# AER-RC/RRTMG_LW

Hardware: AMD Instinct MI355X
Metric: columns/sec, 72-layer profiles (higher is better)
Workload: dtype f64 (transmittance / tfn codes and their LDS table f32); 1 GPU; 1000000 synthetic 72-layer columns, config 'cloudy' (icld=2: rtrnmr max-random overlap, idrv=0), sharded 1x1000000; ncol_total=1000000, nlay=72, columns_per_gpu=1000000, parallelism=columns/1, gather=none, kdata=stand-in (real k-data absent from the reference mount), sweeps=production

## Files before the change

include/rrtmg_lw_hip.h:

```cpp
#ifndef RRTMG_LW_HIP_H
#define RRTMG_LW_HIP_H

#ifdef __cplusplus
extern "C" {
#endif

#define RRTMG_LW_HIP_OK 0
#define RRTMG_LW_HIP_EPHYSICS 1
#define RRTMG_LW_HIP_EARG 2
#define RRTMG_LW_HIP_ENODEVICE 3
#define RRTMG_LW_HIP_ENOTINIT 4
#define RRTMG_LW_HIP_EDATA 5
#define RRTMG_LW_HIP_EHIP 6

#define RRTMG_LW_NBND 16
#define RRTMG_LW_NGPT 140

int rrtmg_lw_hip_init(const char *static_tables_path, const char *kdata_path, double cpdair, int device);

int rrtmg_lw_hip_init_devices(const char *static_tables_path, const char *kdata_path, double cpdair, int ndev, const int *devices);
int rrtmg_lw_hip_num_devices(void);

int rrtmg_lw_hip_kdata_is_standin(void);

// ... 173 lines not shown
    const double *cldfr, const double *taucld, const double *cicewp, const double *cliqwp,
    const double *reice, const double *reliq, const double *tauaer,
    double *uflx, double *dflx, double *hr, double *uflxc, double *dflxc, double *hrc,
    double *duflx_dt, double *duflxc_dt);
int rrtmg_lw_hip_queue_flush(void);
int rrtmg_lw_hip_queue_columns(void);

unsigned rrtmg_lw_hip_build_flags(void);
int rrtmg_lw_hip_set_batch(int ncol_batch);
int rrtmg_lw_hip_effective_batch(int nlay);
int rrtmg_lw_hip_set_overlap(int on);
int rrtmg_lw_hip_set_cu_partition(int layer_cus);
int rrtmg_lw_hip_cu_partition(void);
int rrtmg_lw_hip_set_one_sweep_max(int ncol);
int rrtmg_lw_hip_set_split_max(int ncol);
int rrtmg_lw_hip_set_graph_max(int ncol);
void rrtmg_lw_hip_graph_stats(long long *captures, long long *replays);
int rrtmg_lw_hip_set_wide_window(int on);

int rrtmg_lw_hip_set_layer_split(int on);
int rrtmg_lw_hip_set_column_sort(int on, int min_gain);
int rrtmg_lw_hip_column_sort_min(void);
long long rrtmg_lw_hip_workspace_bytes(void);
int rrtmg_lw_hip_set_n1_prototype(int on);
int rrtmg_lw_hip_n1_prototype(void);
int rrtmg_lw_hip_num_chunks(void);
int rrtmg_lw_hip_gpoints(void);

void rrtmg_lw_hip_profile_begin(void);
int rrtmg_lw_hip_profile_end(char *buf, int len);
// ... 33 lines not shown
```

rrtmg_lw_amd/api.py:

```python
from __future__ import annotations

import ctypes as C
import os

import numpy as np

_HERE = os.path.dirname(os.path.abspath(__file__))
LIB_PATH = os.environ.get("RRTMG_LW_HIP_LIB", os.path.join(_HERE, "librrtmg_lw_hip.so"))
STATIC_BLOB = os.path.join(_HERE, "data", "lw_static.bin")
STANDIN_KDATA = os.path.join(_HERE, "data", "standin.kdata.bin")
REAL_KDATA = os.path.join(os.path.dirname(_HERE), "data", "rrtmg_lw.kdata.bin")
NBND, NGPT = 16, 140

LIB_PATH_G256 = os.path.join(_HERE, "librrtmg_lw_hip_g256.so")

_dp = C.POINTER(C.c_double)
_lib = None
_libs = {}
_gpoints = 140
_initialised = False


class RrtmgLwError(RuntimeError):
    pass
# ... 121 lines not shown
def workspace_bytes():
    lib().rrtmg_lw_hip_workspace_bytes.restype = C.c_longlong
    return int(lib().rrtmg_lw_hip_workspace_bytes())


def set_one_sweep_max(ncol):
    return int(lib().rrtmg_lw_hip_set_one_sweep_max(C.c_int(int(ncol))))


def set_layer_split(on):
    return int(lib().rrtmg_lw_hip_set_layer_split(C.c_int(1 if on else 0)))


def set_split_max(ncol):
    return int(lib().rrtmg_lw_hip_set_split_max(C.c_int(int(ncol))))


def set_graph_max(ncol):
    return int(lib().rrtmg_lw_hip_set_graph_max(C.c_int(int(ncol))))


def graph_stats():
    a, b = C.c_longlong(0), C.c_longlong(0)
    lib().rrtmg_lw_hip_graph_stats(C.byref(a), C.byref(b))
    return int(a.value), int(b.value)


def set_wide_window(on):
    return int(lib().rrtmg_lw_hip_set_wide_window(C.c_int(1 if on else 0)))

# ... 429 lines not shown
```

rrtmg_lw_amd/csrc/driver.hip:

```cpp
#include <hip/hip_runtime.h>
#include <cstdlib>
#include <sched.h>

#include <algorithm>
#include <atomic>
#include <cstdint>
#include <cstdarg>
#include <mutex>
#include <string>
#include <chrono>
#include <condition_variable>
#include <functional>
#include <map>
#include <thread>
#include <vector>

#include "../../include/rrtmg_lw_hip.h"
#include "kernels.hip"
#include "mtjump.hpp"

namespace {

using namespace rrlw;

// ... 214 lines not shown
        } else {                                                                                 \
            hipLaunchKernelGGL(KERNEL, GRID, BLOCKDIM, LDS, STREAM, __VA_ARGS__);                \
        }                                                                                        \
    } while (0)

template <int Q, bool SPEC = false>
int sweepc_attr_one()
{
#ifndef RRLW_TUNE
    HIP_TRY(hipFuncSetAttribute((const void *)k_sweepc<Q, 0, false, sweepc_nt(Q, 0, false), SPEC>, hipFuncAttributeMaxDynamicSharedMemorySize, SWEEPC_LDS_MAX));
    HIP_TRY(hipFuncSetAttribute((const void *)k_sweepc<Q, 0, true, sweepc_nt(Q, 0, true), SPEC>, hipFuncAttributeMaxDynamicSharedMemorySize, SWEEPC_LDS_MAX));
    HIP_TRY(hipFuncSetAttribute((const void *)k_sweepc<Q, 2, true, sweepc_nt(Q, 2, true), SPEC>, hipFuncAttributeMaxDynamicSharedMemorySize, SWEEPC_LDS_MAX));
#endif
    HIP_TRY(hipFuncSetAttribute((const void *)k_sweepc<Q, 1, false, sweepc_nt(Q, 1, false), SPEC>, hipFuncAttributeMaxDynamicSharedMemorySize, SWEEPC_LDS_MAX));
    HIP_TRY(hipFuncSetAttribute((const void *)k_sweepc<Q, 2, false, sweepc_nt(Q, 2, false), SPEC>, hipFuncAttributeMaxDynamicSharedMemorySize, SWEEPC_LDS_MAX));
    return 0;
}
template <int Q>
int sweepz_attr_spec()
{
#ifndef RRLW_TUNE
    HIP_TRY(hipFuncSetAttribute((const void *)k_sweepz<Q, 1, false, true>, hipFuncAttributeMaxDynamicSharedMemorySize, SWEEPC_LDS_MAX));
    HIP_TRY(hipFuncSetAttribute((const void *)k_sweepz<Q, 1, true, true>, hipFuncAttributeMaxDynamicSharedMemorySize, SWEEPC_LDS_MAX));
    HIP_TRY(hipFuncSetAttribute((const void *)k_sweepz<Q, 2, true, true>, hipFuncAttributeMaxDynamicSharedMemorySize, SWEEPC_LDS_MAX));
    HIP_TRY(hipFuncSetAttribute((const void *)k_sweepz<Q, 3, false, true>, hipFuncAttributeMaxDynamicSharedMemorySize, SWEEPC_LDS_MAX));
    HIP_TRY(hipFuncSetAttribute((const void *)k_sweepz<Q, 3, true, true>, hipFuncAttributeMaxDynamicSharedMemorySize, SWEEPC_LDS_MAX));
    HIP_TRY(hipFuncSetAttribute((const void *)k_sweepz<Q, 4, false, true>, hipFuncAttributeMaxDynamicSharedMemorySize, SWEEPC_LDS_MAX));
    HIP_TRY(hipFuncSetAttribute((const void *)k_sweepz<Q, 4, true, true>, hipFuncAttributeMaxDynamicSharedMemorySize, SWEEPC_LDS_MAX));
#endif
    HIP_TRY(hipFuncSetAttribute((const void *)k_sweepz<Q, 2, false, true>, hipFuncAttributeMaxDynamicSharedMemorySize, SWEEPC_LDS_MAX));
// ... 72 lines not shown
        const int zcap = sweepz_group_cap(nq, idrv == 1);
        const int cap = std::max(1, std::min(sweepc_group_cap(nq), mode != 0 ? zcap : 99));
        for (int k0 = 0; k0 < nbs[nq]; k0 += cap) {
            if (fg.n >= NGROUP_MAX) return false;
            const int nbg = std::min(cap, nbs[nq] - k0);
            fg.nb[fg.n] = nbg;
            fg.bands[fg.n] = (lists[nq] >> (4 * k0)) & (nbg >= 16 ? ~0ull : ((1ull << (4 * nbg)) - 1ull));
            fg.gq[fg.n++] = nq;
        }
    }
    return true;
}

void graphs_clear();
int g_split_max = []() { const char *e = getenv("RRTMG_LW_SPLIT_MAX"); return e ? std::max(0, atoi(e)) : 768; }();
int ensure_workspace(int nlay, int ncolb, bool cloud, bool mc = false, int idrv = 1, int mode = -1)
{
    SweepGroups fgw;
    int groups = NGROUP_MAX;
    if (mode >= 0 && make_groups(mode, idrv, 1, NBND, fgw)) groups = fgw.n;
    const bool gdp = idrv == 1, efcl = cloud && (mode < 0 || mode == 1 || mode == 3), ovl = cloud && (mode < 0 || mode == 2);
    const size_t split_cols = ncolb <= g_split_max ? (size_t)NBND * align_up((size_t)ncolb, 64) : 0;
    if (G.ws_base && G.ws_nlay == nlay && G.ws_ncolb >= ncolb && (G.ws_cloud || !cloud) && (G.ws_mc || !mc) && (G.ws_two_scr || !G.split_sweep) &&
        G.ws_groups >= groups && G.ws_slabcols >= split_cols && (G.ws_gdp || !gdp) && (G.ws_efcl || !efcl) && (G.ws_ovl || !ovl)) return 0;
    if (G.ws_base) { HIP_TRY(hipDeviceSynchronize()); graphs_clear(); HIP_TRY(hipFree(G.ws_base)); G.ws_base = nullptr; }
    const bool same = G.ws_nlay == nlay;
    ncolb = std::max(ncolb, same ? G.ws_ncolb : 0);
    cloud = cloud || G.ws_cloud || mc;
    mc = mc || G.ws_mc;
    const int ng = std::max(groups, G.ws_groups);
// ... 285 lines not shown
    sa.tlay = GCM ? g.tlay : c.tavel;
    sa.tlev = GCM ? g.tlev : c.tz;
    const bool spec = GCM && out.uflxs;
    sa.uflxs = spec ? out.uflxs : nullptr; sa.dflxs = spec ? out.dflxs : nullptr;
    sa.uflxcs = spec ? out.uflxcs : nullptr; sa.dflxcs = spec ? out.dflxcs : nullptr;
    SweepGroups fg;
    if (!make_groups(mode, idrv, istart, iend, fg)) return fail(RRTMG_LW_HIP_EARG, "internal: more than %d sweep groups", NGROUP_MAX);
    if ((!split && fg.n > G.ws_groups) || (idrv == 1 && !G.ws_gdp)) return fail(RRTMG_LW_HIP_EARG, "internal: workspace holds %d band groups, the call needs %d", G.ws_groups, fg.n);
    const int *gq = fg.gq;
    int slab0[NGROUP_MAX];
    unsigned long long gsz = 0ull;
    { int sl = 0; for (int g = 0; g < fg.n; g++) { slab0[g] = sl; const int n = split ? fg.nb[g] : 1; gsz |= (unsigned long long)n << (4 * g); sl += n; } }
#define SWEEPC_I(Q, PH, I)                                                                                           \
    do {                                                                                                             \
        constexpr int nt = sweepc_nt(Q, PH, I);                                                                      \
        const int wnb = split ? 1 : sa.nbands;                                             \
        const int nsb = split ? 1 : sweepc_nsb(Q, PH, I, sa.nbands);                                                 \
        sa.ncb = (nb + 64 * nsb - 1) / (64 * nsb);                                                                   \
        const dim3 sgrid((unsigned)sa.ncb, split ? sa.nbands : 1), sblock(64, wnb * nt, nsb);                        \
        if (spec) LAUNCH_LDS("k_sweepc<" #Q "," #PH ",spec>", (k_sweepc<Q, PH, I, nt, true>), sgrid, sblock, sweepc_lds_bytes(PH, I, wnb, nsb, nt), s, G.D, Wk, sa); \
        else LAUNCH_LDS("k_sweepc<" #Q "," #PH ">", (k_sweepc<Q, PH, I, nt>), sgrid, sblock, sweepc_lds_bytes(PH, I, wnb, nsb, nt), s, G.D, Wk, sa); \
    } while (0)
#ifdef RRLW_TUNE
#define SWEEPC(Q, PH) do { if (idrv == 1) return fail(RRTMG_LW_HIP_EARG, "tuning build: idrv = 0 only"); else SWEEPC_I(Q, PH, false); } while (0)
#else
#define SWEEPC(Q, PH) do { if (idrv == 1 && PH != 1) SWEEPC_I(Q, PH, true); else SWEEPC_I(Q, PH, false); } while (0)
#endif
#define SWEEPC_Q(PH) do { if (nq == 4) SWEEPC(4, PH); else if (nq == 3) SWEEPC(3, PH); else if (nq == 2) SWEEPC(2, PH); else SWEEPC(1, PH); } while (0)
    for (int phase = 0; phase < 3; phase++) {
        if (phase == 1) {
            if (mode == 0) continue;
            for (int g = 0; g < fg.n; g++) {
                const int nq = gq[g];
                sa.bands = fg.bands[g];
// ... 169 lines not shown
        if (int rc = make_stream(&G.lay_m, 0, G.cu_layer)) return rc;
    }
    if (G.ev_last_valid) HIP_TRY(hipStreamWaitEvent(s, G.ev_last, 0));
    State::GraphEnt *gent = nullptr;
    bool capture = false;
    if (single && !split && !gen.on && !mc && !G.profile && !G.n1 && ncol <= g_graph_max) {
        std::vector<unsigned char> key;
        key_put(key, ncol); key_put(key, nlay); key_put(key, mode); key_put(key, idrv); key_put(key, inflag); key_put(key, iceflag); key_put(key, liqflag);
        const double *gp[] = {g.play, g.plev, g.tlay, g.tlev, g.tsfc, g.h2ovmr, g.o3vmr, g.co2vmr, g.ch4vmr, g.n2ovmr, g.o2vmr, g.cfc11vmr, g.cfc12vmr,
                              g.cfc22vmr, g.ccl4vmr, g.emis, g.cldfr, g.taucld, g.cicewp, g.cliqwp, g.reice, g.reliq, g.tauaer, g.tauctot,
                              out.uflx, out.dflx, out.hr, out.uflxc, out.dflxc, out.hrc, out.duflx_dt, out.duflxc_dt, out.fnet, out.fnetc,
                              out.uflxs, out.dflxs, out.uflxcs, out.dflxcs};
        key_put(key, gp);
        key_put(key, G.init_gen); key_put(key, G.device);
        key_put(key, G.ws_base); key_put(key, G.ws_bytes); key_put(key, g_colsort); key_put(key, g_colsort_min); key_put(key, g_one_sweep_max);
        key_put(key, g_wide_window); key_put(key, g_layer_split); key_put(key, g_prep_fork); key_put(key, G.sweep_fanout); key_put(key, eff_batch(nlay)); key_put(key, g_split_max);
        for (auto &e : G.graphs) if (e.key == key) { gent = &e; break; }
        if (!gent) {
            if (G.graphs.size() >= GRAPH_CACHE) {
                size_t old = 0;
                for (size_t j = 1; j < G.graphs.size(); j++) if (G.graphs[j].used < G.graphs[old].used) old = j;
                if (G.graphs[old].exec) (void)hipGraphExecDestroy(G.graphs[old].exec);
                G.graphs.erase(G.graphs.begin() + (long)old);
            }
            G.graphs.emplace_back();
            gent = &G.graphs.back();
            gent->key = key;
        }
        gent->used = ++G.graph_clock;
        if (gent->exec) {
            HIP_TRY(hipGraphLaunch(gent->exec, s));
// ... 1119 lines not shown
    g_graph_max = ncol < 0 ? 0 : ncol;
    return prev;
}
void rrtmg_lw_hip_graph_stats(long long *captures, long long *replays)
{
    ENTRY_LOCK;
    if (captures) *captures = g_states[0].graph_captures;
    if (replays) *replays = g_states[0].graph_replays;
}

int rrtmg_lw_hip_set_split_max(int ncol)
{
    ENTRY_LOCK;
    const int prev = g_split_max;
    g_split_max = ncol < 0 ? 0 : ncol;
    return prev;
}

int rrtmg_lw_hip_set_wide_window(int on)
{
    ENTRY_LOCK;
    const int prev = g_wide_window ? 1 : 0;
    g_wide_window = on != 0;
    return prev;
}

int rrtmg_lw_hip_set_layer_split(int on)
{
    ENTRY_LOCK;
    const int prev = g_layer_split ? 1 : 0;
// ... 1304 lines not shown
```

rrtmg_lw_amd/csrc/kernels.hip:

```cpp
#include <hip/hip_runtime.h>
#include "kissjump.hpp"

#if (defined(RRLW_KO_LDS_UNIFORM) || defined(RRLW_KO_HALFG) || defined(RRLW_KO_STORES) || defined(RRLW_KO_HALFSTORE)) && !defined(RRLW_TUNE)
#error "RRLW_KO_* knock-outs give wrong results: tuning builds (-DRRLW_TUNE) only"
#endif
#ifdef RRLW_TUNE
#define RRLW_BF_TUNE 1u
#else
#define RRLW_BF_TUNE 0u
#endif
#if defined(RRLW_KO_LDS_UNIFORM) || defined(RRLW_KO_HALFG) || defined(RRLW_KO_STORES) || defined(RRLW_KO_HALFSTORE)
#define RRLW_BF_KNOCKOUT 2u
#else
#define RRLW_BF_KNOCKOUT 0u
#endif
#if (defined(RRLW_CODE_BITS) && RRLW_CODE_BITS != 32) || defined(RRLW_DECODE_F64) || defined(RRLW_SWEEP_EXPF) || defined(RRLW_EXACT_DIV) || defined(RRLW_FDIV_TWO_NEWTON)
#define RRLW_BF_NUMERICS 4u
#else
#define RRLW_BF_NUMERICS 0u
#endif
#ifdef RRLW_G256
#define RRLW_BF_G256 8u
#else
#define RRLW_BF_G256 0u
// ... 2590 lines not shown
    const float t = (float)idx * 1.0e-4f;
    const float tau = bpade * t * __builtin_amdgcn_rcpf(1.0f - t);
    const float ex = __builtin_amdgcn_exp2f(-1.44269504088896f * tau);
    const float atr = 1.0f - ex;
    float tfn = tau < 0.06f ? tau * (1.0f / 6.0f) : 1.0f - 2.0f * (__builtin_amdgcn_rcpf(tau) - ex * __builtin_amdgcn_rcpf(atr));
    if (idx == 0u) tfn = 0.0f;
    if (idx >= 10000u) tfn = 1.0f;
    return make_float2(idx == 0u ? 0.0f : atr, tfn);
}
#ifdef RRLW_SWEEP_EXPF
#define RRLW_LUT_ENTRY(lut, idx) lut_entry_expf((idx), 3.5971223f)
#else
#define RRLW_LUT_ENTRY(lut, idx) (lut)[(idx)]
#endif

__device__ __forceinline__ double planck_at(const double *tp, const double *tq, double t)
{
    const double x = t - 159.;
    const int ind = clampi((int)x, 1, 180);
    const double f = x - (double)ind;
    return fma(f, tq[ind] - tq[ind - 1], tp[ind - 1]);
}

__device__ __forceinline__ void sweep_stage_lut(const DevTables &T, unsigned char *smem, int tid, int nth)
{
    const double2 *src = reinterpret_cast<const double2 *>(T.stat + T.sl.lutf);
    double2 *dst = reinterpret_cast<double2 *>(smem);
#ifdef RRLW_SWEEP_EXPF
    constexpr int NLUT = 0;
#else
    constexpr int NLUT = SWEEP_LUT_BYTES / 16;
#endif
    for (int i0 = tid; i0 < NLUT; i0 += 8 * nth) {
        double2 v[8];
#pragma unroll
        for (int k = 0; k < 8; k++) v[k] = src[min(i0 + k * nth, NLUT - 1)];
// ... 64 lines not shown
    return (RRLW_SWEEPC_SPLIT && NQ == 4 && (PHASE == 2 || PHASE == 0)) ? 2 : 1;
}
__host__ __device__ constexpr int sweepc_group_cap(int NQ)
{
    int cap = 5;
    for (int ph = 0; ph < 3; ph++)
        for (int i = 0; i < 2; i++) {
            if (ph == 1 && i == 1) continue;
            const bool idrv = i == 1;
            const int nt = sweepc_nt(NQ, ph, idrv), w = 4 * sweepc_waves(NQ / nt, ph, idrv) / nt;
            if (w < cap) cap = w;
            while (cap > 1 && sweepc_lds_bytes(ph, idrv, cap, 1, nt) > SWEEPC_LDS_MAX) cap--;
        }
    return cap;
}
__host__ __device__ constexpr int sweepc_nsb(int NQ, int PHASE, bool IDRV, int nb)
{
    const int nt = sweepc_nt(NQ, PHASE, IDRV);
    int nsb = nsb_fit(4 * sweepc_waves(NQ / nt, PHASE, IDRV) / (nb * nt));
    while (nsb > 1 && sweepc_lds_bytes(PHASE, IDRV, nb, nsb, nt) > SWEEPC_LDS_MAX) nsb = nsb_fit(nsb - 1);
    return nsb;
}

template <int G> struct SweepcLev { double tl, tz; unsigned w; };

__device__ __forceinline__ double one_minus(double x)
{
    double t = 1.0 - x;
    asm("" : "+v"(t));
    return t;
}
__device__ __forceinline__ double times(double x, double y)
{
    double t = x * y;
    asm("" : "+v"(t));
    return t;
}

template <int NQ, int PHASE, bool IDRV, int NT = 1, bool SPEC = false>
__global__ __launch_bounds__(256 * sweepc_waves(NQ / NT, PHASE, IDRV), sweepc_waves(NQ / NT, PHASE, IDRV)) void k_sweepc(DevTables T, Workspace W, SweepArgs a)
{
    static_assert(NQ % NT == 0 && (NT == 1 || NT == 2 || NT == 3), "threads per band");
    constexpr int G = NQ / NT, NG = 4 * G, NC = RRLW_SWEEPC_CODES;
    constexpr bool DOWN = PHASE != 2, UP = PHASE != 1, TWO = PHASE == 2;
    constexpr int NVAL = sweepc_nval(PHASE, IDRV);
    extern __shared__ __align__(16) unsigned char smem[];
    const int tx = threadIdx.x, ty = __builtin_amdgcn_readfirstlane(threadIdx.y), sub = __builtin_amdgcn_readfirstlane(threadIdx.z);
    const int bi = ty / NT, part = ty % NT;
    const int ny = blockDim.y, nb = ny / NT, nsb = blockDim.z, ncw = 64 * nsb;
    const float2 *s_lut = reinterpret_cast<const float2 *>(smem);
    double (*s_pl)[184] = reinterpret_cast<double (*)[184]>(smem + SWEEP_LUT_BYTES + bi * SWEEPC_BAND_BYTES);
    double (*s_fr)[16] = reinterpret_cast<double (*)[16]>(smem + SWEEP_LUT_BYTES + bi * SWEEPC_BAND_BYTES + SWEEP_PL_BYTES);
    double *red = reinterpret_cast<double *>(smem + SWEEP_LUT_BYTES + nb * SWEEPC_BAND_BYTES);
    const int slot = blockIdx.x * nsb + sub;
    const int cblock = PHASE == 0 ? slot : __builtin_amdgcn_readfirstlane(W.order[slot]);
    const int col = cblock * 64 + tx;
    const int bsel = a.split ? (int)blockIdx.y : 0;
    const unsigned long long bands = a.bands >> (4 * bsel);
    const int B = (int)((bands >> (4 * bi)) & 15ull) + 1;
    const bool incol = col < a.ncol;
    const int colc = incol ? col : a.ncol - 1;
    const int quad = __builtin_amdgcn_readfirstlane(band_qstart(B) + part * G);
    const int g0 = NG * part;
    const int pc = pcol(W, colc);
    const size_t gc = (size_t)a.col0 + pc;
    const int nlay = W.nlay, nct = a.nct;
    const size_t ncb = W.ncolb;
    const bool alt16 = (B == 16 && a.istart == 16);
    const bool lo_bin = (LO_BINARY >> (B - 1)) & 1u, up_bin = (UP_BINARY >> (B - 1)) & 1u;
    const bool any_bin = lo_bin || up_bin;
    const int base_up = ((UP_ZERO >> (B - 1)) & 1u) ? 14 : (((UP_FROM_A >> (B - 1)) & 1u) ? 0 : 9);
    sweep_stage_lut(T, smem, (sub * ny + ty) * 64 + tx, 64 * ny * nsb);
    sweep_stage_band(T, s_pl, s_fr, B, alt16, lo_bin, up_bin, (sub * NT + part) * 64 + tx, NT * ncw);
    __syncthreads();
    const int lo = PHASE == 0 ? 1 : __builtin_amdgcn_readfirstlane(W.hgrp[(blockIdx.x * nsb) / SORT_GROUP]) + 1;
    const size_t qstride = (size_t)nlay * ncb;
    const unsigned *__restrict__ sC = W.scr[S_CODE] + (size_t)quad * qstride * CODE_WORDS;
    const unsigned *__restrict__ sFw = W.fw + (size_t)fw_slot(B) * nlay * ncb;
    const bool moved = pmoved(W, colc);
    const double *__restrict__ tlay = moved ? W.tlayc : a.tlay + a.col0;
    const double *__restrict__ tlev = moved ? W.tlevc : a.tlev + a.col0;
    const size_t tstride = moved ? ncb : (size_t)nct;
    const unsigned offc = (unsigned)colc * (unsigned)CODE_BYTES, off8p = (unsigned)colc * 8u, off4 = (unsigned)colc * 4u;
    const size_t pcb = (size_t)W.pcb;
    const size_t gslab = (size_t)(a.group + bsel) * (nlay + 1) * pcb;
    double *__restrict__ gdn1 = W.gdn1 + gslab;
    double *__restrict__ gup1 = W.gup1 + gslab;
    Part2 *__restrict__ gup = W.gup + gslab;
    Part2 *__restrict__ gdp = W.gdp + gslab;
    const unsigned so8 = (unsigned)col * 8u, so16 = (unsigned)col * 16u;
    const int laytrop = W.laytrop[colc];
    const double *tp0 = s_pl[0], *tp1 = s_pl[1];
    double2 *hand = reinterpret_cast<double2 *>(W.hand) + ((size_t)quad * ncb + colc) * 2;
    const size_t hstream = (size_t)NQUAD * ncb * 2;

    constexpr bool SOFF = PHASE != 1;
    const unsigned ncb32 = (unsigned)ncb, tstr32 = (unsigned)tstride;
    auto fill_t = [&](auto bin_tag, int lev, int zoff, SweepcLev<G> &q) {
        const int l = min(max(lev, 1), nlay);
        if constexpr (SOFF) {
            const unsigned r = (unsigned)(l - 1);
            q.tl = bload_f64(row_ptr(tlay, r, tstr32), off8p);
            q.tz = bload_f64(row_ptr(tlev, r + (unsigned)zoff, tstr32), off8p);
            if constexpr (decltype(bin_tag)::value) q.w = bload_u32(sFw, off4, r * ncb32 * 4u);
        } else {
            q.tl = bload_f64(tlay + tstride * (l - 1), off8p);
            q.tz = bload_f64(tlev + tstride * (l - 1 + zoff), off8p);
            if constexpr (decltype(bin_tag)::value) q.w = bload_u32(sFw + (size_t)(l - 1) * ncb, off4);
        }
    };
    auto ld_c = [&](int lev, int k) -> pk4 {
        const int l = min(max(lev, 1), nlay);
        if constexpr (SOFF) return bload_pk4_nt(sC + (size_t)k * qstride * CODE_WORDS, offc, (unsigned)(l - 1) * ncb32 * (unsigned)CODE_BYTES);
        else return bload_pk4_nt(sC + ((size_t)k * qstride + (size_t)(l - 1) * ncb) * CODE_WORDS, offc);
    };
    auto frac_row = [&](int lev, unsigned fwv, double &fpl) -> const double * {
        const bool lower = lev <= laytrop;
        if (any_bin) {
            const unsigned w = (lower ? lo_bin : up_bin) ? fwv : 0x10000000u;
            const int r0 = clampi((lower ? 0 : base_up) + (int)(w >> 28) - 1, 0, 14);
            fpl = (double)(w & 0x0fffffffu) * (1.0 / 268435456.0);
            return &s_fr[r0][g0];
        }
        fpl = 0.0;
        return &s_fr[lower ? 0 : base_up][g0];
    };

    const unsigned rlane = (unsigned)(sub * 64 + tx);
    const unsigned vstride = (unsigned)(ny * NC * ncw), rband = (unsigned)(ty * NC * ncw);
    unsigned bufoff = 0u;
    auto red_put = [&](int c, int val, double v) { red[bufoff + val * vstride + rband + (unsigned)(c * ncw) + rlane] = v; };
    auto round_end = [&](auto dn_tag, int lev0, int nvalid) {
#pragma clang fp contract(off)
        constexpr bool DN = decltype(dn_tag)::value;
        constexpr int NV = DN ? 1 : NVAL;
        __syncthreads();
        for (int c = ty; c < nvalid; c += ny) {
            const int lvl = DN ? lev0 - c - 1 : lev0 + c;
            double sv[NV];
#pragma unroll
            for (int val = 0; val < NV; val++) {
                const double *r = red + (bufoff + val * vstride + (unsigned)(c * ncw) + rlane);
                const bool deriv = IDRV && !DN && val >= (TWO ? 2 : 1);
                double sum = 0.0;
                for (int q = 0; q < nb; q++) {
                    double pq = r[(unsigned)(q * NT * NC * ncw)];
// ... 19 lines not shown
                if constexpr (DN) bstore_f64(gdn1 + (size_t)lvl * pcb, so8, sv[0]);
                else {
                    if constexpr (TWO) bstore_f64x2(gup + (size_t)lvl * pcb, so16, sv[0], sv[1]);
                    else bstore_f64(gup1 + (size_t)lvl * pcb, so8, sv[0]);
                    if constexpr (IDRV) bstore_f64x2(gdp + (size_t)lvl * pcb, so16, TWO ? sv[2] : sv[1], TWO ? sv[3] : sv[1]);
                }
            }
        }
        bufoff = bufoff ? 0u : NVAL * vstride;
    };

    double rad[NG], radc[TWO ? NG : 1], drad[IDRV ? NG : 1], dradc[(IDRV && TWO) ? NG : 1];
#pragma unroll
    for (int j = 0; j < NG; j++) rad[j] = 0.0;

    SweepcLev<G> cur;
    cur.w = 0u;
    pk4 cc[G][NC];
    int ki = 0;
    auto level = [&](auto bin_tag, auto dn_tag, int lev, int slot) {
        constexpr bool BIN = decltype(bin_tag)::value, DN = decltype(dn_tag)::value;
        constexpr int dir = DN ? -1 : 1;
        ki_salu(ki);
        double fpl;
        const double *row = frac_row(lev, cur.w, fpl);
        const double blay = planck_at(tp0, tp0, cur.tl);
        const double dpl = planck_at(tp0, (DN && alt16 && lev == 1) ? tp1 : tp0, cur.tz) - blay;
        fill_t(bin_tag, lev + dir, DN ? 0 : 1, cur);
        double qs[G], qsc[G], qd[G], qdc[G];
#pragma unroll
        for (int k = 0; k < G; k++) {
            float2 e[4];
            pk4 pk;
#pragma unroll
            for (int c = 0; c < NC; c++) if (c == slot) pk = cc[k][c];
            const scr4 ck = unpack4(pk);
#pragma unroll
            for (int jj = 0; jj < 4; jj++) e[jj] = RRLW_LUT_ENTRY(s_lut, code_index(ck.v[jj]));
            {
                const pk4 nx = ld_c(lev + NC * dir, k);
#pragma unroll
                for (int c = 0; c < NC; c++) if (c == slot) cc[k][c] = nx;
            }
#pragma unroll
            for (int jj = 0; jj < 4; jj++) {
                const int j = 4 * k + jj;
                double atr, tfn;
                decode(ck.v[jj], e[jj], atr, tfn);
                double fr = row[j];
                if constexpr (BIN) fr = fma(fpl, row[16 + j] - fr, fr);
                const double bb = fr * fma(tfn, dpl, blay);
                rad[j] = fma(bb - rad[j], atr, rad[j]);
                if constexpr (TWO && !DN) radc[j] = fma(bb - radc[j], atr, radc[j]);
                if constexpr (IDRV && !DN) {
                    const double tr = one_minus(atr);
                    drad[j] = times(drad[j], tr);
                    if constexpr (TWO) dradc[j] = times(dradc[j], tr);
                }
            }
            qs[k] = (rad[4 * k] + rad[4 * k + 1]) + (rad[4 * k + 2] + rad[4 * k + 3]);
            if constexpr (TWO && !DN) qsc[k] = (radc[4 * k] + radc[4 * k + 1]) + (radc[4 * k + 2] + radc[4 * k + 3]);
            if constexpr (IDRV && !DN) {
                qd[k] = (drad[4 * k] + drad[4 * k + 1]) + (drad[4 * k + 2] + drad[4 * k + 3]);
                if constexpr (TWO) qdc[k] = (dradc[4 * k] + dradc[4 * k + 1]) + (dradc[4 * k + 2] + dradc[4 * k + 3]);
            }
            if (RRLW_SWEEPC_QUAD_BARRIER) __builtin_amdgcn_sched_barrier(0);
        }
        auto tree = [&](const double (&q)[G]) -> double {
            if constexpr (G == 1) return q[0];
            else if constexpr (G == 2) return q[0] + q[1];
            else if constexpr (G == 3) return (q[0] + q[1]) + q[2];
            else return (q[0] + q[1]) + (q[2] + q[3]);
        };
        red_put(slot, 0, tree(qs));
        if constexpr (TWO && !DN) red_put(slot, 1, tree(qsc));
        if constexpr (IDRV && !DN) {
            red_put(slot, TWO ? 2 : 1, tree(qd));
            if constexpr (TWO) red_put(slot, 3, tree(qdc));
        }
    };
    auto sweep = [&](auto bin_tag, auto dn_tag) {
        constexpr bool DN = decltype(dn_tag)::value;
        constexpr int dir = DN ? -1 : 1;
        const int first = DN ? nlay : lo, count = nlay - lo + 1;
#pragma unroll
        for (int c = 0; c < NC; c++) {
            if (c == NC - 1) fill_t(bin_tag, first, DN ? 0 : 1, cur);
#pragma unroll
            for (int k = 0; k < G; k++) cc[k][c] = ld_c(first + c * dir, k);
        }
        int n = 0;
        for (; n + NC <= count; n += NC) {
#pragma unroll
// ... 2 lines not shown
        }
        const int rem = count - n;
#pragma unroll
        for (int c = 0; c < NC - 1; c++) {
            if (c < rem) level(bin_tag, dn_tag, first + (n + c) * dir, c);
        }
        if (rem > 0) round_end(dn_tag, first + n * dir, rem);
    };
    using std::true_type;
    using std::false_type;

    if constexpr (DOWN) {
        if (incol && ty == 0) bstore_f64(gdn1 + (size_t)nlay * pcb, so8, 0.0);
        if constexpr (SPEC) {
            if (incol && part == 0) {
                const size_t o = spec_at(gc, nlay, B, nlay, nct);
                a.dflxs[o] = 0.0;
                if (a.dflxcs) a.dflxcs[o] = 0.0;
            }
        }
        if (any_bin) sweep(true_type{}, true_type{}); else sweep(false_type{}, true_type{});
    }
    if constexpr (PHASE == 1) {
        if (incol) {
#pragma unroll
            for (int k = 0; k < G; k++) {
                hand[(size_t)k * ncb * 2] = make_double2(rad[4 * k], rad[4 * k + 1]);
                hand[(size_t)k * ncb * 2 + 1] = make_double2(rad[4 * k + 2], rad[4 * k + 3]);
            }
        }
        return;
    }

    if constexpr (PHASE == 0) {
        const double reflect = 1. - a.emis[gc + (size_t)nct * (B - 1)];
        const double pb = W.percol[(size_t)(PC_PLANKBND + B - 1) * ncb + colc];
        const double dpb = IDRV ? W.percol[(size_t)(PC_DPLANKBND + B - 1) * ncb + colc] : 0.0;
        double fpl;
        const double *row = frac_row(1, any_bin ? bload_u32(sFw, off4) : 0u, fpl);
        double usum = 0.0, dusum = 0.0;
#pragma unroll
        for (int j = 0; j < NG; j++) {
            const double fr = any_bin ? fma(fpl, row[16 + j] - row[j], row[j]) : row[j];
            rad[j] = fma(reflect, rad[j], fr * pb);
            usum = usum + rad[j];
            if constexpr (IDRV) { drad[j] = times(fr, dpb); dusum = dusum + drad[j]; }
        }
        red_put(0, 0, usum);
        if constexpr (IDRV) red_put(0, 1, dusum);
        round_end(false_type{}, 0, 1);
    } else {
#pragma unroll
        for (int k = 0; k < G; k++) {
            const double2 *h = hand + (size_t)k * ncb * 2;
            const double2 a0 = h[hstream], a1 = h[hstream + 1], c0 = h[2 * hstream], c1 = h[2 * hstream + 1];
            rad[4 * k] = a0.x; rad[4 * k + 1] = a0.y; rad[4 * k + 2] = a1.x; rad[4 * k + 3] = a1.y;
            if constexpr (TWO) { radc[4 * k] = c0.x; radc[4 * k + 1] = c0.y; radc[4 * k + 2] = c1.x; radc[4 * k + 3] = c1.y; }
            if constexpr (IDRV) {
                const double2 d0 = h[3 * hstream], d1 = h[3 * hstream + 1], e0 = h[4 * hstream], e1 = h[4 * hstream + 1];
                drad[4 * k] = d0.x; drad[4 * k + 1] = d0.y; drad[4 * k + 2] = d1.x; drad[4 * k + 3] = d1.y;
                if constexpr (TWO) { dradc[4 * k] = e0.x; dradc[4 * k + 1] = e0.y; dradc[4 * k + 2] = e1.x; dradc[4 * k + 3] = e1.y; }
            }
        }
    }
    if constexpr (UP) {
        if (any_bin) sweep(true_type{}, false_type{}); else sweep(false_type{}, false_type{});
    }
}

// ... 740 lines not shown
```

Baseline: 17.27 million columns/s.

## Merge several single-quad bands per thread in the clear-sky sweep kernel

```diff
diff --git a/include/rrtmg_lw_hip.h b/include/rrtmg_lw_hip.h
--- a/include/rrtmg_lw_hip.h
+++ b/include/rrtmg_lw_hip.h
@@ -211,6 +211,7 @@
 int rrtmg_lw_hip_cu_partition(void);
 int rrtmg_lw_hip_set_one_sweep_max(int ncol);
 int rrtmg_lw_hip_set_split_max(int ncol);
+int rrtmg_lw_hip_set_band_merge(int on);
 int rrtmg_lw_hip_set_graph_max(int ncol);
 void rrtmg_lw_hip_graph_stats(long long *captures, long long *replays);
 int rrtmg_lw_hip_set_wide_window(int on);
diff --git a/rrtmg_lw_amd/api.py b/rrtmg_lw_amd/api.py
--- a/rrtmg_lw_amd/api.py
+++ b/rrtmg_lw_amd/api.py
@@ -159,6 +159,10 @@
 
 def set_split_max(ncol):
     return int(lib().rrtmg_lw_hip_set_split_max(C.c_int(int(ncol))))
+
+
+def set_band_merge(on):
+    return int(lib().rrtmg_lw_hip_set_band_merge(C.c_int(1 if on else 0)))
 
 
 def set_graph_max(ncol):
diff --git a/rrtmg_lw_amd/csrc/driver.hip b/rrtmg_lw_amd/csrc/driver.hip
--- a/rrtmg_lw_amd/csrc/driver.hip
+++ b/rrtmg_lw_amd/csrc/driver.hip
@@ -252,6 +252,15 @@
 #endif
     HIP_TRY(hipFuncSetAttribute((const void *)k_sweepc<Q, 1, false, sweepc_nt(Q, 1, false), SPEC>, hipFuncAttributeMaxDynamicSharedMemorySize, SWEEPC_LDS_MAX));
     HIP_TRY(hipFuncSetAttribute((const void *)k_sweepc<Q, 2, false, sweepc_nt(Q, 2, false), SPEC>, hipFuncAttributeMaxDynamicSharedMemorySize, SWEEPC_LDS_MAX));
+    if constexpr (!SPEC && sweepc_nbt(Q, 1, false) > 1) {
+#ifndef RRLW_TUNE
+        HIP_TRY(hipFuncSetAttribute((const void *)k_sweepc<Q, 0, false, 1, false, sweepc_nbt(Q, 0, false)>, hipFuncAttributeMaxDynamicSharedMemorySize, SWEEPC_LDS_MAX));
+        HIP_TRY(hipFuncSetAttribute((const void *)k_sweepc<Q, 0, true, 1, false, sweepc_nbt(Q, 0, true)>, hipFuncAttributeMaxDynamicSharedMemorySize, SWEEPC_LDS_MAX));
+        HIP_TRY(hipFuncSetAttribute((const void *)k_sweepc<Q, 2, true, 1, false, sweepc_nbt(Q, 2, true)>, hipFuncAttributeMaxDynamicSharedMemorySize, SWEEPC_LDS_MAX));
+#endif
+        HIP_TRY(hipFuncSetAttribute((const void *)k_sweepc<Q, 1, false, 1, false, sweepc_nbt(Q, 1, false)>, hipFuncAttributeMaxDynamicSharedMemorySize, SWEEPC_LDS_MAX));
+        HIP_TRY(hipFuncSetAttribute((const void *)k_sweepc<Q, 2, false, 1, false, sweepc_nbt(Q, 2, false)>, hipFuncAttributeMaxDynamicSharedMemorySize, SWEEPC_LDS_MAX));
+    }
     return 0;
 }
 template <int Q>
@@ -354,6 +363,8 @@
 
 void graphs_clear();
 int g_split_max = []() { const char *e = getenv("RRTMG_LW_SPLIT_MAX"); return e ? std::max(0, atoi(e)) : 768; }();
+constexpr int bands_with_quads(int nq) { int n = 0; for (int B = 1; B <= NBND; B++) n += band_nquad(B) == nq ? 1 : 0; return n; }
+bool g_band_merge = []() { const char *e = getenv("RRTMG_LW_BAND_MERGE"); return !e || atoi(e) != 0; }();
 int ensure_workspace(int nlay, int ncolb, bool cloud, bool mc = false, int idrv = 1, int mode = -1)
 {
     SweepGroups fgw;
@@ -669,10 +680,15 @@
 #define SWEEPC_I(Q, PH, I)                                                                                           \
     do {                                                                                                             \
         constexpr int nt = sweepc_nt(Q, PH, I);                                                                      \
+        constexpr int nbt = sweepc_nbt(Q, PH, I);                                 \
+        const bool merge = nbt > 1 && g_band_merge && !split && !spec && sa.nbands == bands_with_quads(Q);             \
         const int wnb = split ? 1 : sa.nbands;                                             \
-        const int nsb = split ? 1 : sweepc_nsb(Q, PH, I, sa.nbands);                                                 \
+        const int nsb = split ? 1 : sweepc_nsb(Q, PH, I, sa.nbands, merge ? nbt : 1);                                \
         sa.ncb = (nb + 64 * nsb - 1) / (64 * nsb);                                                                   \
-        const dim3 sgrid((unsigned)sa.ncb, split ? sa.nbands : 1), sblock(64, wnb * nt, nsb);                        \
+        const dim3 sgrid((unsigned)sa.ncb, split ? sa.nbands : 1), sblock(64, merge ? wnb / nbt : wnb * nt, nsb);    \
+        if constexpr (nbt > 1) {                                                                                     \
+            if (merge) { LAUNCH_LDS("k_sweepc<" #Q "," #PH ",merged>", (k_sweepc<Q, PH, I, 1, false, nbt>), sgrid, sblock, sweepc_lds_bytes(PH, I, wnb, nsb, 1), s, G.D, Wk, sa); break; } \
+        }                                                                                                            \
         if (spec) LAUNCH_LDS("k_sweepc<" #Q "," #PH ",spec>", (k_sweepc<Q, PH, I, nt, true>), sgrid, sblock, sweepc_lds_bytes(PH, I, wnb, nsb, nt), s, G.D, Wk, sa); \
         else LAUNCH_LDS("k_sweepc<" #Q "," #PH ">", (k_sweepc<Q, PH, I, nt>), sgrid, sblock, sweepc_lds_bytes(PH, I, wnb, nsb, nt), s, G.D, Wk, sa); \
     } while (0)
@@ -872,7 +888,7 @@
         key_put(key, gp);
         key_put(key, G.init_gen); key_put(key, G.device);
         key_put(key, G.ws_base); key_put(key, G.ws_bytes); key_put(key, g_colsort); key_put(key, g_colsort_min); key_put(key, g_one_sweep_max);
-        key_put(key, g_wide_window); key_put(key, g_layer_split); key_put(key, g_prep_fork); key_put(key, G.sweep_fanout); key_put(key, eff_batch(nlay)); key_put(key, g_split_max);
+        key_put(key, g_wide_window); key_put(key, g_layer_split); key_put(key, g_prep_fork); key_put(key, G.sweep_fanout); key_put(key, eff_batch(nlay)); key_put(key, g_split_max); key_put(key, g_band_merge);
         for (auto &e : G.graphs) if (e.key == key) { gent = &e; break; }
         if (!gent) {
             if (G.graphs.size() >= GRAPH_CACHE) {
@@ -2022,6 +2038,14 @@
     ENTRY_LOCK;
     const int prev = g_split_max;
     g_split_max = ncol < 0 ? 0 : ncol;
+    return prev;
+}
+
+int rrtmg_lw_hip_set_band_merge(int on)
+{
+    ENTRY_LOCK;
+    const int prev = g_band_merge ? 1 : 0;
+    g_band_merge = on != 0;
     return prev;
 }
 
diff --git a/rrtmg_lw_amd/csrc/kernels.hip b/rrtmg_lw_amd/csrc/kernels.hip
--- a/rrtmg_lw_amd/csrc/kernels.hip
+++ b/rrtmg_lw_amd/csrc/kernels.hip
@@ -2628,12 +2628,22 @@
 #define RRLW_LUT_ENTRY(lut, idx) (lut)[(idx)]
 #endif
 
+__device__ __forceinline__ void planck_idx(double t, int &ind, double &f)
+{
+    const double x = t - 159.;
+    ind = clampi((int)x, 1, 180);
+    f = x - (double)ind;
+}
+__device__ __forceinline__ double planck_eval(const double *tp, const double *tq, int ind, double f)
+{
+    return fma(f, tq[ind] - tq[ind - 1], tp[ind - 1]);
+}
 __device__ __forceinline__ double planck_at(const double *tp, const double *tq, double t)
 {
-    const double x = t - 159.;
-    const int ind = clampi((int)x, 1, 180);
-    const double f = x - (double)ind;
-    return fma(f, tq[ind] - tq[ind - 1], tp[ind - 1]);
+    int ind;
+    double f;
+    planck_idx(t, ind, f);
+    return planck_eval(tp, tq, ind, f);
 }
 
 __device__ __forceinline__ void sweep_stage_lut(const DevTables &T, unsigned char *smem, int tid, int nth)
@@ -2728,15 +2738,22 @@
         }
     return cap;
 }
-__host__ __device__ constexpr int sweepc_nsb(int NQ, int PHASE, bool IDRV, int nb)
+__host__ __device__ constexpr int sweepc_nbt(int NQ, int PHASE, bool IDRV) { (void)IDRV; return NQ != 1 ? 1 : PHASE == 1 ? 4 : 2; }
+__host__ __device__ constexpr int sweepc_waves_m(int PHASE, bool IDRV) { return PHASE == 0 && !IDRV ? 3 : 2; }
+__host__ __device__ constexpr int sweepc_waves_of(int NQ, int PHASE, bool IDRV, int NT, int NBT)
+{
+    return NBT == 1 ? sweepc_waves(NQ / NT, PHASE, IDRV) : sweepc_waves_m(PHASE, IDRV);
+}
+__host__ __device__ constexpr int sweepc_nsb(int NQ, int PHASE, bool IDRV, int nb, int NBT = 1)
 {
     const int nt = sweepc_nt(NQ, PHASE, IDRV);
-    int nsb = nsb_fit(4 * sweepc_waves(NQ / nt, PHASE, IDRV) / (nb * nt));
-    while (nsb > 1 && sweepc_lds_bytes(PHASE, IDRV, nb, nsb, nt) > SWEEPC_LDS_MAX) nsb = nsb_fit(nsb - 1);
+    int nsb = NBT == 1 ? nsb_fit(4 * sweepc_waves(NQ / nt, PHASE, IDRV) / (nb * nt))
+                       : nsb_fit(4 * sweepc_waves_m(PHASE, IDRV) / (nb / NBT));
+    while (nsb > 1 && sweepc_lds_bytes(PHASE, IDRV, nb, nsb, NBT == 1 ? nt : 1) > SWEEPC_LDS_MAX) nsb = nsb_fit(nsb - 1);
     return nsb;
 }
 
-template <int G> struct SweepcLev { double tl, tz; unsigned w; };
+template <int NB> struct SweepcLev { double tl, tz; unsigned w[NB]; };
 
 __device__ __forceinline__ double one_minus(double x)
 {
@@ -2751,46 +2768,59 @@
     return t;
 }
 
-template <int NQ, int PHASE, bool IDRV, int NT = 1, bool SPEC = false>
-__global__ __launch_bounds__(256 * sweepc_waves(NQ / NT, PHASE, IDRV), sweepc_waves(NQ / NT, PHASE, IDRV)) void k_sweepc(DevTables T, Workspace W, SweepArgs a)
+template <int NQ, int PHASE, bool IDRV, int NT = 1, bool SPEC = false, int NBT = 1>
+__global__ __launch_bounds__(256 * sweepc_waves_of(NQ, PHASE, IDRV, NT, NBT), sweepc_waves_of(NQ, PHASE, IDRV, NT, NBT)) void k_sweepc(DevTables T, Workspace W, SweepArgs a)
 {
     static_assert(NQ % NT == 0 && (NT == 1 || NT == 2 || NT == 3), "threads per band");
-    constexpr int G = NQ / NT, NG = 4 * G, NC = RRLW_SWEEPC_CODES;
+    static_assert(NBT == 1 || (NT == 1 && !SPEC), "several bands per thread: whole bands, no spectral outputs");
+    constexpr int G = NQ * NBT / NT, NG = 4 * G, QB = G / NBT, NC = RRLW_SWEEPC_CODES;
     constexpr bool DOWN = PHASE != 2, UP = PHASE != 1, TWO = PHASE == 2;
     constexpr int NVAL = sweepc_nval(PHASE, IDRV);
     extern __shared__ __align__(16) unsigned char smem[];
     const int tx = threadIdx.x, ty = __builtin_amdgcn_readfirstlane(threadIdx.y), sub = __builtin_amdgcn_readfirstlane(threadIdx.z);
-    const int bi = ty / NT, part = ty % NT;
-    const int ny = blockDim.y, nb = ny / NT, nsb = blockDim.z, ncw = 64 * nsb;
+    const int bi = (ty / NT) * NBT, part = ty % NT;
+    const int ny = blockDim.y, nb = (ny / NT) * NBT, nsb = blockDim.z, ncw = 64 * nsb;
     const float2 *s_lut = reinterpret_cast<const float2 *>(smem);
-    double (*s_pl)[184] = reinterpret_cast<double (*)[184]>(smem + SWEEP_LUT_BYTES + bi * SWEEPC_BAND_BYTES);
-    double (*s_fr)[16] = reinterpret_cast<double (*)[16]>(smem + SWEEP_LUT_BYTES + bi * SWEEPC_BAND_BYTES + SWEEP_PL_BYTES);
     double *red = reinterpret_cast<double *>(smem + SWEEP_LUT_BYTES + nb * SWEEPC_BAND_BYTES);
     const int slot = blockIdx.x * nsb + sub;
     const int cblock = PHASE == 0 ? slot : __builtin_amdgcn_readfirstlane(W.order[slot]);
     const int col = cblock * 64 + tx;
     const int bsel = a.split ? (int)blockIdx.y : 0;
     const unsigned long long bands = a.bands >> (4 * bsel);
-    const int B = (int)((bands >> (4 * bi)) & 15ull) + 1;
     const bool incol = col < a.ncol;
     const int colc = incol ? col : a.ncol - 1;
-    const int quad = __builtin_amdgcn_readfirstlane(band_qstart(B) + part * G);
     const int g0 = NG * part;
     const int pc = pcol(W, colc);
     const size_t gc = (size_t)a.col0 + pc;
     const int nlay = W.nlay, nct = a.nct;
     const size_t ncb = W.ncolb;
-    const bool alt16 = (B == 16 && a.istart == 16);
-    const bool lo_bin = (LO_BINARY >> (B - 1)) & 1u, up_bin = (UP_BINARY >> (B - 1)) & 1u;
-    const bool any_bin = lo_bin || up_bin;
-    const int base_up = ((UP_ZERO >> (B - 1)) & 1u) ? 14 : (((UP_FROM_A >> (B - 1)) & 1u) ? 0 : 9);
+    int B[NBT], quad[NBT], base_up[NBT];
+    bool alt16[NBT], lo_bin[NBT], up_bin[NBT], any_bin = false;
+    double (*s_pl[NBT])[184];
+    double (*s_fr[NBT])[16];
     sweep_stage_lut(T, smem, (sub * ny + ty) * 64 + tx, 64 * ny * nsb);
-    sweep_stage_band(T, s_pl, s_fr, B, alt16, lo_bin, up_bin, (sub * NT + part) * 64 + tx, NT * ncw);
+#pragma unroll
+    for (int kb = 0; kb < NBT; kb++) {
+        B[kb] = (int)((bands >> (4 * (bi + kb))) & 15ull) + 1;
+        quad[kb] = __builtin_amdgcn_readfirstlane(band_qstart(B[kb]) + part * G);
+        alt16[kb] = (B[kb] == 16 && a.istart == 16);
+        lo_bin[kb] = (LO_BINARY >> (B[kb] - 1)) & 1u;
+        up_bin[kb] = (UP_BINARY >> (B[kb] - 1)) & 1u;
+        any_bin = any_bin || lo_bin[kb] || up_bin[kb];
+        base_up[kb] = ((UP_ZERO >> (B[kb] - 1)) & 1u) ? 14 : (((UP_FROM_A >> (B[kb] - 1)) & 1u) ? 0 : 9);
+        s_pl[kb] = reinterpret_cast<double (*)[184]>(smem + SWEEP_LUT_BYTES + (bi + kb) * SWEEPC_BAND_BYTES);
+        s_fr[kb] = reinterpret_cast<double (*)[16]>(smem + SWEEP_LUT_BYTES + (bi + kb) * SWEEPC_BAND_BYTES + SWEEP_PL_BYTES);
+        sweep_stage_band(T, s_pl[kb], s_fr[kb], B[kb], alt16[kb], lo_bin[kb], up_bin[kb], (sub * NT + part) * 64 + tx, NT * ncw);
+    }
     __syncthreads();
     const int lo = PHASE == 0 ? 1 : __builtin_amdgcn_readfirstlane(W.hgrp[(blockIdx.x * nsb) / SORT_GROUP]) + 1;
     const size_t qstride = (size_t)nlay * ncb;
-    const unsigned *__restrict__ sC = W.scr[S_CODE] + (size_t)quad * qstride * CODE_WORDS;
-    const unsigned *__restrict__ sFw = W.fw + (size_t)fw_slot(B) * nlay * ncb;
+    const unsigned *sC[NBT], *sFw[NBT];
+#pragma unroll
+    for (int kb = 0; kb < NBT; kb++) {
+        sC[kb] = W.scr[S_CODE] + (size_t)quad[kb] * qstride * CODE_WORDS;
+        sFw[kb] = W.fw + (size_t)(NBT == 1 ? fw_slot(B[kb]) : min(fw_slot(B[kb]), NFW - 1)) * nlay * ncb;
+    }
     const bool moved = pmoved(W, colc);
     const double *__restrict__ tlay = moved ? W.tlayc : a.tlay + a.col0;
     const double *__restrict__ tlev = moved ? W.tlevc : a.tlev + a.col0;
@@ -2804,46 +2834,52 @@
     Part2 *__restrict__ gdp = W.gdp + gslab;
     const unsigned so8 = (unsigned)col * 8u, so16 = (unsigned)col * 16u;
     const int laytrop = W.laytrop[colc];
-    const double *tp0 = s_pl[0], *tp1 = s_pl[1];
-    double2 *hand = reinterpret_cast<double2 *>(W.hand) + ((size_t)quad * ncb + colc) * 2;
+    auto hand_at = [&](int k) -> double2 * { return reinterpret_cast<double2 *>(W.hand) + ((size_t)(quad[k / QB] + k % QB) * ncb + colc) * 2; };
     const size_t hstream = (size_t)NQUAD * ncb * 2;
 
     constexpr bool SOFF = PHASE != 1;
     const unsigned ncb32 = (unsigned)ncb, tstr32 = (unsigned)tstride;
-    auto fill_t = [&](auto bin_tag, int lev, int zoff, SweepcLev<G> &q) {
+    auto fill_t = [&](auto bin_tag, int lev, int zoff, SweepcLev<NBT> &q) {
         const int l = min(max(lev, 1), nlay);
         if constexpr (SOFF) {
             const unsigned r = (unsigned)(l - 1);
             q.tl = bload_f64(row_ptr(tlay, r, tstr32), off8p);
             q.tz = bload_f64(row_ptr(tlev, r + (unsigned)zoff, tstr32), off8p);
-            if constexpr (decltype(bin_tag)::value) q.w = bload_u32(sFw, off4, r * ncb32 * 4u);
+            if constexpr (decltype(bin_tag)::value) {
+#pragma unroll
+                for (int kb = 0; kb < NBT; kb++) q.w[kb] = bload_u32(sFw[kb], off4, r * ncb32 * 4u);
+            }
         } else {
             q.tl = bload_f64(tlay + tstride * (l - 1), off8p);
             q.tz = bload_f64(tlev + tstride * (l - 1 + zoff), off8p);
-            if constexpr (decltype(bin_tag)::value) q.w = bload_u32(sFw + (size_t)(l - 1) * ncb, off4);
+            if constexpr (decltype(bin_tag)::value) {
+#pragma unroll
+                for (int kb = 0; kb < NBT; kb++) q.w[kb] = bload_u32(sFw[kb] + (size_t)(l - 1) * ncb, off4);
+            }
         }
     };
     auto ld_c = [&](int lev, int k) -> pk4 {
         const int l = min(max(lev, 1), nlay);
-        if constexpr (SOFF) return bload_pk4_nt(sC + (size_t)k * qstride * CODE_WORDS, offc, (unsigned)(l - 1) * ncb32 * (unsigned)CODE_BYTES);
-        else return bload_pk4_nt(sC + ((size_t)k * qstride + (size_t)(l - 1) * ncb) * CODE_WORDS, offc);
+        const unsigned *c0 = sC[k / QB];
+        if constexpr (SOFF) return bload_pk4_nt(c0 + (size_t)(k % QB) * qstride * CODE_WORDS, offc, (unsigned)(l - 1) * ncb32 * (unsigned)CODE_BYTES);
+        else return bload_pk4_nt(c0 + ((size_t)(k % QB) * qstride + (size_t)(l - 1) * ncb) * CODE_WORDS, offc);
     };
-    auto frac_row = [&](int lev, unsigned fwv, double &fpl) -> const double * {
+    auto frac_row = [&](int kb, int lev, unsigned fwv, double &fpl) -> const double * {
         const bool lower = lev <= laytrop;
         if (any_bin) {
-            const unsigned w = (lower ? lo_bin : up_bin) ? fwv : 0x10000000u;
-            const int r0 = clampi((lower ? 0 : base_up) + (int)(w >> 28) - 1, 0, 14);
+            const unsigned w = (lower ? lo_bin[kb] : up_bin[kb]) ? fwv : 0x10000000u;
+            const int r0 = clampi((lower ? 0 : base_up[kb]) + (int)(w >> 28) - 1, 0, 14);
             fpl = (double)(w & 0x0fffffffu) * (1.0 / 268435456.0);
-            return &s_fr[r0][g0];
+            return &s_fr[kb][r0][g0];
         }
         fpl = 0.0;
-        return &s_fr[lower ? 0 : base_up][g0];
+        return &s_fr[kb][lower ? 0 : base_up[kb]][g0];
     };
 
     const unsigned rlane = (unsigned)(sub * 64 + tx);
-    const unsigned vstride = (unsigned)(ny * NC * ncw), rband = (unsigned)(ty * NC * ncw);
+    const unsigned vstride = (unsigned)(ny * NBT * NC * ncw), rband = (unsigned)(ty * NBT * NC * ncw);
     unsigned bufoff = 0u;
-    auto red_put = [&](int c, int val, double v) { red[bufoff + val * vstride + rband + (unsigned)(c * ncw) + rlane] = v; };
+    auto red_put = [&](int c, int val, double v, int kb = 0) { red[bufoff + val * vstride + rband + (unsigned)((kb * NC + c) * ncw) + rlane] = v; };
     auto round_end = [&](auto dn_tag, int lev0, int nvalid) {
 #pragma clang fp contract(off)
         constexpr bool DN = decltype(dn_tag)::value;
@@ -2893,18 +2929,30 @@
 #pragma unroll
     for (int j = 0; j < NG; j++) rad[j] = 0.0;
 
-    SweepcLev<G> cur;
-    cur.w = 0u;
+    SweepcLev<NBT> cur;
+#pragma unroll
+    for (int kb = 0; kb < NBT; kb++) cur.w[kb] = 0u;
     pk4 cc[G][NC];
     int ki = 0;
     auto level = [&](auto bin_tag, auto dn_tag, int lev, int slot) {
         constexpr bool BIN = decltype(bin_tag)::value, DN = decltype(dn_tag)::value;
         constexpr int dir = DN ? -1 : 1;
         ki_salu(ki);
-        double fpl;
-        const double *row = frac_row(lev, cur.w, fpl);
-        const double blay = planck_at(tp0, tp0, cur.tl);
-        const double dpl = planck_at(tp0, (DN && alt16 && lev == 1) ? tp1 : tp0, cur.tz) - blay;
+        double fpl[NBT], blay[NBT], dpl[NBT];
+        const double *row[NBT];
+        {
+            int il, iz;
+            double fl, fz;
+            planck_idx(cur.tl, il, fl);
+            planck_idx(cur.tz, iz, fz);
+#pragma unroll
+            for (int kb = 0; kb < NBT; kb++) {
+                const double *tp0 = s_pl[kb][0], *tp1 = s_pl[kb][1];
+                row[kb] = frac_row(kb, lev, cur.w[kb], fpl[kb]);
+                blay[kb] = planck_eval(tp0, tp0, il, fl);
+                dpl[kb] = planck_eval(tp0, (DN && alt16[kb] && lev == 1) ? tp1 : tp0, iz, fz) - blay[kb];
+            }
+        }
         fill_t(bin_tag, lev + dir, DN ? 0 : 1, cur);
         double qs[G], qsc[G], qd[G], qdc[G];
 #pragma unroll
@@ -2923,12 +2971,12 @@
             }
 #pragma unroll
             for (int jj = 0; jj < 4; jj++) {
-                const int j = 4 * k + jj;
+                const int j = 4 * k + jj, kb = k / QB, jb = 4 * (k % QB) + jj;
                 double atr, tfn;
                 decode(ck.v[jj], e[jj], atr, tfn);
-                double fr = row[j];
-                if constexpr (BIN) fr = fma(fpl, row[16 + j] - fr, fr);
-                const double bb = fr * fma(tfn, dpl, blay);
+                double fr = row[kb][jb];
+                if constexpr (BIN) fr = fma(fpl[kb], row[kb][16 + jb] - fr, fr);
+                const double bb = fr * fma(tfn, dpl[kb], blay[kb]);
                 rad[j] = fma(bb - rad[j], atr, rad[j]);
                 if constexpr (TWO && !DN) radc[j] = fma(bb - radc[j], atr, radc[j]);
                 if constexpr (IDRV && !DN) {
@@ -2945,17 +2993,21 @@
             }
             if (RRLW_SWEEPC_QUAD_BARRIER) __builtin_amdgcn_sched_barrier(0);
         }
-        auto tree = [&](const double (&q)[G]) -> double {
-            if constexpr (G == 1) return q[0];
-            else if constexpr (G == 2) return q[0] + q[1];
-            else if constexpr (G == 3) return (q[0] + q[1]) + q[2];
-            else return (q[0] + q[1]) + (q[2] + q[3]);
+        auto tree = [&](const double (&q)[G], int kb) -> double {
+            const int o = kb * QB;
+            if constexpr (QB == 1) return q[o];
+            else if constexpr (QB == 2) return q[o] + q[o + 1];
+            else if constexpr (QB == 3) return (q[o] + q[o + 1]) + q[o + 2];
+            else return (q[o] + q[o + 1]) + (q[o + 2] + q[o + 3]);
         };
-        red_put(slot, 0, tree(qs));
-        if constexpr (TWO && !DN) red_put(slot, 1, tree(qsc));
-        if constexpr (IDRV && !DN) {
-            red_put(slot, TWO ? 2 : 1, tree(qd));
-            if constexpr (TWO) red_put(slot, 3, tree(qdc));
+#pragma unroll
+        for (int kb = 0; kb < NBT; kb++) {
+            red_put(slot, 0, tree(qs, kb), kb);
+            if constexpr (TWO && !DN) red_put(slot, 1, tree(qsc, kb), kb);
+            if constexpr (IDRV && !DN) {
+                red_put(slot, TWO ? 2 : 1, tree(qd, kb), kb);
+                if constexpr (TWO) red_put(slot, 3, tree(qdc, kb), kb);
+            }
         }
     };
     auto sweep = [&](auto bin_tag, auto dn_tag) {
@@ -2988,7 +3040,7 @@
         if (incol && ty == 0) bstore_f64(gdn1 + (size_t)nlay * pcb, so8, 0.0);
         if constexpr (SPEC) {
             if (incol && part == 0) {
-                const size_t o = spec_at(gc, nlay, B, nlay, nct);
+                const size_t o = spec_at(gc, nlay, B[0], nlay, nct);
                 a.dflxs[o] = 0.0;
                 if (a.dflxcs) a.dflxcs[o] = 0.0;
             }
@@ -2999,34 +3051,39 @@
         if (incol) {
 #pragma unroll
             for (int k = 0; k < G; k++) {
-                hand[(size_t)k * ncb * 2] = make_double2(rad[4 * k], rad[4 * k + 1]);
-                hand[(size_t)k * ncb * 2 + 1] = make_double2(rad[4 * k + 2], rad[4 * k + 3]);
+                double2 *h = hand_at(k);
+                h[0] = make_double2(rad[4 * k], rad[4 * k + 1]);
+                h[1] = make_double2(rad[4 * k + 2], rad[4 * k + 3]);
             }
         }
         return;
     }
 
     if constexpr (PHASE == 0) {
-        const double reflect = 1. - a.emis[gc + (size_t)nct * (B - 1)];
-        const double pb = W.percol[(size_t)(PC_PLANKBND + B - 1) * ncb + colc];
-        const double dpb = IDRV ? W.percol[(size_t)(PC_DPLANKBND + B - 1) * ncb + colc] : 0.0;
-        double fpl;
-        const double *row = frac_row(1, any_bin ? bload_u32(sFw, off4) : 0u, fpl);
-        double usum = 0.0, dusum = 0.0;
-#pragma unroll
-        for (int j = 0; j < NG; j++) {
-            const double fr = any_bin ? fma(fpl, row[16 + j] - row[j], row[j]) : row[j];
-            rad[j] = fma(reflect, rad[j], fr * pb);
-            usum = usum + rad[j];
-            if constexpr (IDRV) { drad[j] = times(fr, dpb); dusum = dusum + drad[j]; }
-        }
-        red_put(0, 0, usum);
-        if constexpr (IDRV) red_put(0, 1, dusum);
+#pragma unroll
+        for (int kb = 0; kb < NBT; kb++) {
+            const double reflect = 1. - a.emis[gc + (size_t)nct * (B[kb] - 1)];
+            const double pb = W.percol[(size_t)(PC_PLANKBND + B[kb] - 1) * ncb + colc];
+            const double dpb = IDRV ? W.percol[(size_t)(PC_DPLANKBND + B[kb] - 1) * ncb + colc] : 0.0;
+            double fpl;
+            const double *row = frac_row(kb, 1, any_bin ? bload_u32(sFw[kb], off4) : 0u, fpl);
+            double usum = 0.0, dusum = 0.0;
+#pragma unroll
+            for (int jb = 0; jb < 4 * QB; jb++) {
+                const int j = 4 * QB * kb + jb;
+                const double fr = any_bin ? fma(fpl, row[16 + jb] - row[jb], row[jb]) : row[jb];
+                rad[j] = fma(reflect, rad[j], fr * pb);
+                usum = usum + rad[j];
+                if constexpr (IDRV) { drad[j] = times(fr, dpb); dusum = dusum + drad[j]; }
+            }
+            red_put(0, 0, usum, kb);
+            if constexpr (IDRV) red_put(0, 1, dusum, kb);
+        }
         round_end(false_type{}, 0, 1);
     } else {
 #pragma unroll
         for (int k = 0; k < G; k++) {
-            const double2 *h = hand + (size_t)k * ncb * 2;
+            const double2 *h = hand_at(k);
             const double2 a0 = h[hstream], a1 = h[hstream + 1], c0 = h[2 * hstream], c1 = h[2 * hstream + 1];
             rad[4 * k] = a0.x; rad[4 * k + 1] = a0.y; rad[4 * k + 2] = a1.x; rad[4 * k + 3] = a1.y;
             if constexpr (TWO) { radc[4 * k] = c0.x; radc[4 * k + 1] = c0.y; radc[4 * k + 2] = c1.x; radc[4 * k + 3] = c1.y; }
```

Measured after the change: 17.26 million columns/s, median of 2. No clear change (-0.1%).
